# uurl/hivemq-mqtt-tensorflow-kafka-realtime-iot-machine-learning-training-inference

Hardware: AMD Instinct MI355X
Metric: sensor-rows/sec (autoencoder train) + p50 per-event inference µs at 1/2/4/8 MI355X (higher is better)
Workload: dtype bf16

## Files before the change

### hivemq-mqtt-tensorflow-kafka-realtime-iot-machine-learning-training-inference_amd/csrc/include/sml_common.h

```cpp
#pragma once
#include <hip/hip_runtime.h>
#include <stdint.h>

#if defined(SML_KERNEL_CHECKS) && SML_KERNEL_CHECKS
#define SML_DCHECK(cond)                                                           \
  do {                                                                             \
    if (!(cond)) {                                                                 \
      printf("SML_DCHECK failed: %s (%s:%d)\n", #cond, __FILE__, __LINE__);        \
      __builtin_trap();                                                            \
    }                                                                              \
  } while (0)
#else
#define SML_DCHECK(cond) ((void)0)
#endif

namespace sml {

typedef short bf16x4 __attribute__((ext_vector_type(4)));
typedef float f32x4 __attribute__((ext_vector_type(4)));
typedef __bf16 bf16x2_t __attribute__((ext_vector_type(2)));
typedef float f32x2_t __attribute__((ext_vector_type(2)));

enum Act : int { ACT_LINEAR = 0, ACT_RELU = 1, ACT_TANH = 2, ACT_SIGMOID = 3 };

// ... 72 lines not shown
    case ACT_TANH: return 1.0f - h * h;
    case ACT_SIGMOID: return h * (1.0f - h);
    default: return 1.0f;
  }
}

__device__ __forceinline__ bf16x4 identity_b(int c, int g) {
  bf16x4 r;
#pragma unroll
  for (int j = 0; j < 4; ++j) r[j] = (4 * g + j == c) ? (short)0x3F80 : (short)0;
  return r;
}

__device__ __forceinline__ f32x4 transpose_tile(bf16x4 t, bf16x4 ident) {
  f32x4 z = {0.f, 0.f, 0.f, 0.f};
  return mfma16(t, ident, z);
}

__device__ __forceinline__ float xor16(float v, int lane) {
  const unsigned u = __float_as_uint(v);
  const auto r = __builtin_amdgcn_permlane16_swap(u, u, false, false);
  return __uint_as_float(((lane >> 4) & 1) ? r[0] : r[1]);
}
__device__ __forceinline__ float xor32(float v, int lane) {
  const unsigned u = __float_as_uint(v);
  const auto r = __builtin_amdgcn_permlane32_swap(u, u, false, false);
  return __uint_as_float(lane >= 32 ? r[0] : r[1]);
}
__device__ __forceinline__ int xor16i(int v, int lane) { return __float_as_int(xor16(__int_as_float(v), lane)); }
__device__ __forceinline__ int xor32i(int v, int lane) { return __float_as_int(xor32(__int_as_float(v), lane)); }

typedef __attribute__((address_space(3))) bf16x4 lds_bf16x4;

__device__ __forceinline__ int tr_wr_off(int c, int g) { return c * 32 + 8 * (g ^ ((c >> 2) & 3)); }
__device__ __forceinline__ int tr_rd_off(int c, int g) { return (4 * g + (c >> 2)) * 32 + 8 * ((c & 3) ^ g); }
__device__ __forceinline__ bf16x4 lds_transpose(bf16x4 v, char* wave_scratch, int c, int g) {
  lds_bf16x4* wr = (lds_bf16x4*)(wave_scratch + tr_wr_off(c, g));
  *wr = v;
  lds_bf16x4* rd = (lds_bf16x4*)(wave_scratch + tr_rd_off(c, g));
  return __builtin_amdgcn_ds_read_tr16_b64_v4i16(rd);
}

__device__ __forceinline__ float wave_sum(float v) {
#pragma unroll
  for (int o = 32; o > 0; o >>= 1) v += __shfl_xor(v, o, 64);
  return v;
}

}
```

### hivemq-mqtt-tensorflow-kafka-realtime-iot-machine-learning-training-inference_amd/csrc/kernels/ae_fused.hip

```cpp
#include <cstdlib>

#include "sml_common.h"
#include "sml_adam.h"

using namespace sml;

namespace {

constexpr int WAVES = 4;
constexpr int OFF1 = 0, OFF2 = 512, OFF3 = 768, OFF4 = 1024;
constexpr int NPARAM = 1536;
constexpr int NSLOT = 1540;
constexpr int SLAB_BYTES = WAVES * NSLOT * 4;

struct AEArgs {
  const float* x;
  int64_t n;
  int64_t ld;
  const float* scale;
  const float* shift;
  const float* params;
  float* partials;
  int64_t* iter;
  const int64_t* cursor;
// ... 765 lines not shown
  if (s < OFF3) {
    const int in = (s - OFF2) >> 4, out = (s - OFF2) & 15;
    if (out < 7) s2 = s + 8;
    else s1 = -1;
    return;
  }
  const bool l3 = s < OFF4;
  const int base = l3 ? OFF3 : OFF4, w = l3 ? 16 : 32;
  const int in = (s - base) / w, out = (s - base) % w;
  const int pin = in < 7 ? in : (in == 15 ? 7 : -1);
  if (pin < 0 || (l3 && out >= 7)) {
    s1 = -1;
    return;
  }
  if (!l3 && out >= 16) {
    if (out >= 18) {
      s1 = -1;
      return;
    }
    s1 = base + pin * w + 16 + 4 * (out - 16);
    s2 = base + (pin + 8) * w + 16 + 8 + 4 * (out - 16);
    return;
  }
  s1 = base + pin * w + out;
  s2 = base + (pin + 8) * w + out + (l3 ? 8 : 0);
}

__device__ __forceinline__ void tr_write(bf16x4 v, char* slot, int c, int g) {
  *(lds_bf16x4*)(slot + tr_wr_off(c, g)) = v;
}
__device__ __forceinline__ bf16x4 tr_read(char* slot, int c, int g) {
  return __builtin_amdgcn_ds_read_tr16_b64_v4i16((lds_bf16x4*)(slot + tr_rd_off(c, g)));
}

template <int PACK, int DC, bool TP, int TS = 10, int NP = 1, int XP = 0, bool RX = false, bool CM = false,
          bool WA = false, bool RC = true>
__device__ __forceinline__ void train_pair_packed(const AEArgs& a, const FragsP& F, char* scr, int c, int g,
                                                  const f32x4 (&xf)[NP][2][2], const float (&xup)[NP],
                                                  const int (&ix)[NP][2], f32x4 acc1[2], f32x4& acc2, f32x4& acc3,
                                                  f32x4 acc4[2], f32x4& acc2b, f32x4& acc4b, float& sq, float& ab,
                                                  float& corr, float& rows, lds_cc* const* xrow = nullptr,
                                                  lds_cc* const* xupa = nullptr) {
  static_assert(PACK == PACK_REF && DC == 18, "reference model, D = 18 (outputs 16, 17 packed as UP)");
  static_assert(NP == 1 || NP == 2, "one or two pairs per iteration");
  const f32x4 zero4 = {0.f, 0.f, 0.f, 0.f};
  const bf16x4 zb = {0, 0, 0, 0};
  const bool pad_lane = (g == 3);
  const bool lo = c < 8;
  auto stand_in = [](int p, int u) { return TP && p == NP - 1 && u == 1; };
  constexpr bool EW = XP == 1 || XP >= 3, MA = XP >= 1, TRM = XP == 2;
  constexpr bool EB = XP == 4;
  bf16x4 ident;
#pragma unroll
  for (int j = 0; j < 4; ++j) ident[j] = bfbits(4 * g + j == c ? 1.0f : 0.0f);
  auto mfma_tr = [&](bf16x4 v) -> bf16x4 { return pack4(mfma16(v, ident, zero4)); };

  bf16x4 xb0[NP][2], h1b[NP][2], xub[NP];
  f32x4 h1[NP][2], y[NP][2], z1[NP][2], l1s[NP][2];
#pragma unroll
  for (int p = 0; p < NP; ++p) {
#pragma unroll
    for (int u = 0; u < 2; ++u) xb0[p][u] = pack4(xf[p][u][0]);
    xub[p] = pack4(f32x4{xup[p], g == 0 ? 1.0f : 0.0f, 0.f, 0.f});
    if constexpr (EW) {
      tr_write(xb0[p][0], scr + (p * TS + 0) * 512, c, g);
      tr_write(xb0[p][1], scr + (p * TS + 1) * 512, c, g);
      tr_write(xub[p], scr + (p * TS + 2) * 512, c, g);
    }
  }
#pragma unroll
  for (int p = 0; p < NP; ++p) {
    if constexpr (MA) {
      typedef unsigned u32x2 __attribute__((ext_vector_type(2)));
      const unsigned xw = __builtin_bit_cast(u32x2, xub[p])[0];
      const unsigned bias_w = __float_as_uint(g == 0 ? 1.0f : 0.0f);
      const bf16x4 xu0 = __builtin_bit_cast(bf16x4, u32x2{g < 2 ? xw : 0u, 0u});
      const bf16x4 xu1 = __builtin_bit_cast(bf16x4, u32x2{g >= 2 ? xw : bias_w, 0u});
      z1[p][0] = mfma32a(F.w1s, xb0[p][0], xu0, zero4);
      z1[p][1] = mfma32a(F.w1s, xb0[p][1], xu1, zero4);
    } else {
      z1[p][0] = mfma32a(F.w1a[0], xb0[p][0], xub[p], zero4);
      z1[p][1] = mfma32a(F.w1a[1], xub[p], xb0[p][1], zero4);
    }
  }
#pragma unroll
  for (int p = 0; p < NP; ++p)
#pragma unroll
    for (int u = 0; u < 2; ++u) {
#pragma unroll
      for (int i = 0; i < 4; ++i) h1[p][u][i] = tanh_exp2(z1[p][u][i]);
      h1b[p][u] = pack4(h1[p][u]);
      if constexpr (EW) tr_write(h1b[p][u], scr + (p * TS + 3 + u) * 512, c, g);
    }
  auto l1_sign = [&] {
#pragma unroll
    for (int p = 0; p < NP; ++p)
#pragma unroll
      for (int u = 0; u < 2; ++u)
#pragma unroll
        for (int i = 0; i < 4; ++i) l1s[p][u][i] = stand_in(p, u) ? 0.f : __builtin_amdgcn_fmed3f(h1[p][u][i], -a.l1, a.l1);
  };
  if constexpr (!MA) l1_sign();
  f32x4 z2[NP], h2[NP], h3[NP], z3[NP];
  bf16x4 h2b[NP], h3b[NP];
#pragma unroll
  for (int p = 0; p < NP; ++p) z2[p] = mfma32a(F.w2a, h1b[p][0], h1b[p][1], zero4);
#pragma unroll
  for (int p = 0; p < NP; ++p) {
#pragma unroll
    for (int i = 0; i < 4; ++i) h2[p][i] = relu_fast(z2[p][i]);
    h2b[p] = pack4(h2[p]);
    if constexpr (EW) tr_write(h2b[p], scr + (p * TS + 5) * 512, c, g);
  }
#pragma unroll
  for (int p = 0; p < NP; ++p) z3[p] = mfma16(F.w3t, h2b[p], zero4);
#pragma unroll
  for (int p = 0; p < NP; ++p) {
#pragma unroll
    for (int i = 0; i < 4; ++i) h3[p][i] = tanh_exp2(z3[p][i]);
    h3b[p] = pack4(h3[p]);
    if constexpr (EW) tr_write(h3b[p], scr + (p * TS + 6) * 512, c, g);
  }
  f32x4 dz4[NP][2], z4[NP][2], z4u[NP];
  float dz4up[NP], yup[NP];
  f32x4 xl[NP][2];
  float xul[NP];
#pragma unroll
  for (int p = 0; p < NP; ++p) {
    if constexpr (RX) {
      typedef __attribute__((address_space(3))) const float lds_f;
      constexpr int DR = CM ? 14 : 18, SLOTB = 64 * DR + 16;
#pragma unroll
      for (int u = 0; u < 2; ++u) xl[p][u] = ring_row4(xrow[p] + u * SLOTB);
      xul[p] = *(lds_f*)xupa[p];
    } else {
#pragma unroll
      for (int u = 0; u < 2; ++u) xl[p][u] = xf[p][u][0];
      xul[p] = xup[p];
    }
  }
  const float cm_m[3] = {g < 2 ? 0.f : 1.f, g == 1 ? 0.f : 1.f, g == 0 ? 0.f : 1.f};
#pragma unroll
  for (int p = 0; p < NP; ++p) {
#pragma unroll
    for (int u = 0; u < 2; ++u) z4[p][u] = mfma16(F.w4t[u], h3b[p], zero4);
    z4u[p] = mfma16(F.w4u, h3b[p], zero4);
  }
#pragma unroll
  for (int p = 0; p < NP; ++p) {
#pragma unroll
    for (int u = 0; u < 2; ++u)
#pragma unroll
      for (int i = 0; i < 4; ++i) {
        y[p][u][i] = relu_fast(z4[p][u][i]);
        float e = (CM && i < 3) ? fmaf(-xl[p][u][i], cm_m[i], y[p][u][i]) : y[p][u][i] - xl[p][u][i];
        if (stand_in(p, u)) e = 0.f;
        sq = fmaf(e, e, sq);
        dz4[p][u][i] = y[p][u][i] > 0.f ? e : 0.f;
      }
    yup[p] = relu_fast(z4u[p][0]);
    float eup = yup[p] - xul[p];
    if (TP && p == NP - 1) eup = g < 2 ? eup : 0.f;
    sq = fmaf(eup, eup, sq);
    dz4up[p] = yup[p] > 0.f ? eup : 0.f;
  }
  if (WA || a.want_acc) {
#pragma unroll
    for (int p = 0; p < NP; ++p) {
      const int iy = row_argmax_up_pair(y[p][0], y[p][1], yup[p], g);
      const int sel = -(g & 1);
      const int ixs = (ix[p][0] & ~sel) | (ix[p][1] & sel);
      corr += (((TP && p == NP - 1) ? g == 0 : g < 2) && iy == ixs) ? 1.f : 0.f;
    }
  }
  if constexpr (RC) rows += (g == 0) ? (TP ? 2.f * NP - 1.f : 2.f * NP) : 0.f;

  bf16x4 dz4b[NP][2], dz1b[NP][2], dz4bu[NP], dz3b[NP], dz2b[NP];
  f32x4 d3[NP], d2[NP];
#pragma unroll
  for (int p = 0; p < NP; ++p) {
#pragma unroll
    for (int u = 0; u < 2; ++u) dz4b[p][u] = pack4(dz4[p][u]);
    dz4bu[p] = pack4(f32x4{dz4up[p], 0.f, 0.f, 0.f});
    if constexpr (EB) {
      tr_write(dz4b[p][0], scr + (p * TS + 7) * 512, c, g);
      tr_write(dz4b[p][1], scr + (p * TS + 8) * 512, c, g);
      tr_write(dz4bu[p], scr + (p * TS + 9) * 512, c, g);
    }
  }
#pragma unroll
  for (int p = 0; p < NP; ++p) {
    d3[p] = mfma32a(F.w4ba, dz4b[p][0], dz4b[p][1], zero4);
    d3[p] = mfma32a(F.w4bua, dz4bu[p], zb, d3[p]);
  }
#pragma unroll
  for (int p = 0; p < NP; ++p) {
    f32x4 dz3;
#pragma unroll
    for (int i = 0; i < 4; ++i) dz3[i] = d3[p][i] * fmaf(-h3[p][i], h3[p][i], 1.0f);
    dz3b[p] = pack4(dz3);
    if constexpr (EB) tr_write(dz3b[p], scr + (p * TS + 10) * 512, c, g);
  }
#pragma unroll
  for (int p = 0; p < NP; ++p) d2[p] = mfma16(F.w3b, dz3b[p], zero4);
#pragma unroll
  for (int p = 0; p < NP; ++p) {
    f32x4 dz2;
#pragma unroll
    for (int i = 0; i < 4; ++i) dz2[i] = h2[p][i] > 0.f ? d2[p][i] : 0.f;
    dz2b[p] = pack4(dz2);
    if constexpr (EB) tr_write(dz2b[p], scr + (p * TS + 11) * 512, c, g);
  }
  f32x4 d1[NP][2];
  if constexpr (MA) l1_sign();
#pragma unroll
  for (int p = 0; p < NP; ++p)
#pragma unroll
    for (int u = 0; u < 2; ++u) d1[p][u] = mfma16(F.w2b[u], dz2b[p], l1s[p][u]);
#pragma unroll
  for (int p = 0; p < NP; ++p)
#pragma unroll
    for (int u = 0; u < 2; ++u) {
      f32x4 dz1;
#pragma unroll
      for (int i = 0; i < 4; ++i) {
        const float hv = h1[p][u][i];
        if (stand_in(p, u)) {
          dz1[i] = 0.f;
          continue;
        }
        ab += (i == 3 && pad_lane) ? 0.f : fabsf(hv);
        dz1[i] = d1[p][u][i] * fmaf(-hv, hv, 1.0f);
      }
      dz1b[p][u] = pack4(dz1);
    }

  static_assert(TS >= 1 && TS <= 12 && (!EW || TS == (EB ? 12 : 10)), "transpose slots");
  (void)mfma_tr;
#pragma unroll
  for (int p = 0; p < NP; ++p) {
    char* sp = scr + p * TS * 512;
    bf16x4 xr0[2], dz1r[2], h1r[2], dz4r[2], xur, dz4ru, dz2r, h2r, dz3r, h3r;
    if constexpr (EB) {
      h3r = tr_read(sp + 6 * 512, c, g);
      dz4r[0] = tr_read(sp + 7 * 512, c, g);
      dz4r[1] = tr_read(sp + 8 * 512, c, g);
      dz4ru = tr_read(sp + 9 * 512, c, g);
      h2r = tr_read(sp + 5 * 512, c, g);
      dz3r = tr_read(sp + 10 * 512, c, g);
      h1r[0] = tr_read(sp + 3 * 512, c, g);
      h1r[1] = tr_read(sp + 4 * 512, c, g);
      dz2r = tr_read(sp + 11 * 512, c, g);
      xr0[0] = tr_read(sp + 0 * 512, c, g);
      xr0[1] = tr_read(sp + 1 * 512, c, g);
      xur = tr_read(sp + 2 * 512, c, g);
      dz1r[0] = mfma_tr(dz1b[p][0]);
      dz1r[1] = mfma_tr(dz1b[p][1]);
    } else if constexpr (TRM) {
      xr0[0] = mfma_tr(xb0[p][0]);
      xr0[1] = mfma_tr(xb0[p][1]);
      xur = mfma_tr(xub[p]);
      h1r[0] = mfma_tr(h1b[p][0]);
      h1r[1] = mfma_tr(h1b[p][1]);
      h2r = mfma_tr(h2b[p]);
      h3r = mfma_tr(h3b[p]);
      dz4r[0] = mfma_tr(dz4b[p][0]);
      dz4r[1] = mfma_tr(dz4b[p][1]);
      dz4ru = mfma_tr(dz4bu[p]);
      dz3r = mfma_tr(dz3b[p]);
      dz2r = mfma_tr(dz2b[p]);
      dz1r[0] = mfma_tr(dz1b[p][0]);
      dz1r[1] = mfma_tr(dz1b[p][1]);
    } else if constexpr (EW) {
      xr0[0] = tr_read(sp + 0 * 512, c, g);
      xr0[1] = tr_read(sp + 1 * 512, c, g);
      xur = tr_read(sp + 2 * 512, c, g);
// ... 4 lines not shown
      if constexpr (XP == 3) {
        dz4r[0] = mfma_tr(dz4b[p][0]);
        dz4r[1] = mfma_tr(dz4b[p][1]);
        dz4ru = mfma_tr(dz4bu[p]);
        dz3r = mfma_tr(dz3b[p]);
        dz2r = mfma_tr(dz2b[p]);
        dz1r[0] = mfma_tr(dz1b[p][0]);
        dz1r[1] = mfma_tr(dz1b[p][1]);
      } else {
        dz4r[0] = lds_transpose(dz4b[p][0], sp + 7 * 512, c, g);
        dz4r[1] = lds_transpose(dz4b[p][1], sp + 8 * 512, c, g);
        dz4ru = lds_transpose(dz4bu[p], sp + 9 * 512, c, g);
        dz3r = lds_transpose(dz3b[p], sp + 7 * 512, c, g);
        dz2r = lds_transpose(dz2b[p], sp + 8 * 512, c, g);
        dz1r[0] = lds_transpose(dz1b[p][0], sp + 9 * 512, c, g);
        dz1r[1] = lds_transpose(dz1b[p][1], sp + 7 * 512, c, g);
      }
    } else {
      xur = lds_transpose(xub[p], sp + (1 % TS) * 512, c, g);
#pragma unroll
      for (int u = 0; u < 2; ++u) {
        xr0[u] = lds_transpose(xb0[p][u], sp + (0 % TS) * 512, c, g);
        dz1r[u] = lds_transpose(dz1b[p][u], sp + (2 % TS) * 512, c, g);
        h1r[u] = lds_transpose(h1b[p][u], sp + (3 % TS) * 512, c, g);
        dz4r[u] = lds_transpose(dz4b[p][u], sp + (8 % TS) * 512, c, g);
      }
      dz4ru = lds_transpose(dz4bu[p], sp + (9 % TS) * 512, c, g);
      dz2r = lds_transpose(dz2b[p], sp + (4 % TS) * 512, c, g);
      h2r = lds_transpose(h2b[p], sp + (5 % TS) * 512, c, g);
      dz3r = lds_transpose(dz3b[p], sp + (6 % TS) * 512, c, g);
      h3r = lds_transpose(h3b[p], sp + (7 % TS) * 512, c, g);
    }
    acc1[0] = mfma32(xr0[0], xr0[1], dz1r[0], dz1r[1], acc1[0]);
    acc1[1] = mfma32(lo ? xur : zb, (!lo || c == 1) ? xur : zb, dz1r[0], dz1r[1], acc1[1]);
    if constexpr (MA) {
      acc2 = mfma32(h1r[0], h1r[1], lo ? dz2r : zb, lo ? zb : dz2r, acc2);
      acc3 = mfma16(h2r, dz3r, acc3);
      acc4[0] = mfma32(lo ? h3r : zb, lo ? zb : h3r, dz4r[0], dz4r[1], acc4[0]);
    } else {
      acc2 = mfma16(h1r[0], dz2r, acc2);
      acc2b = mfma16(h1r[1], dz2r, acc2b);
      acc3 = mfma16(h2r, dz3r, acc3);
      acc4[0] = mfma16(h3r, dz4r[0], acc4[0]);
      acc4b = mfma16(h3r, dz4r[1], acc4b);
    }
    acc4[1] = mfma16(h3r, dz4ru, acc4[1]);
  }
}

template <int OCC, int ILP = 1>
constexpr int ring_bytes() { return ILP == 3 ? (OCC >= 4 ? 4672 : 7008) : OCC >= 4 ? 3968 : (ILP >= 2 ? 7008 : 6144); }
template <int OCC, int ILP, int PF, int CM = 0>
constexpr int ring_bytes_pf() { return ILP == 3 ? PF * (CM ? 912 : 1168) : ring_bytes<OCC, ILP>(); }

template <int PF, int OCC, int ILP, int TS, int NPW = 1, int CM = 0>
struct AELds {
  static constexpr int SCR = (ILP == 3 ? NPW * TS : 10) * 512;
  static constexpr int NORM_OFF = ILP == 3 ? WAVES * SCR : SLAB_BYTES;
  static constexpr int RING_OFF = NORM_OFF + NORM_BYTES;
  static constexpr int RING = ring_bytes_pf<OCC, ILP, PF, CM>();
  static constexpr int END = RING_OFF + (PF > 0 ? WAVES * RING : 0);
  static constexpr int BYTES = END > SLAB_BYTES ? END : SLAB_BYTES;
};

template <int PACK, bool VEC, int PF, int OCC, int DC = 0, int XM = 0, int ILP = 1, int TS = 10, int NPW = 1,
          int XP = 0, int CM = 0>
__global__ __launch_bounds__(WAVES * 64, OCC) void ae_train_kernel(AEArgs a) {
  constexpr bool FAST = zero_preserving<PACK>();
  constexpr bool CMP = CM != 0;
  static_assert(!CMP || (ILP == 3 && XM == 1 && DC == 18), "compact ring: packed pairs, tile-packed ring, D = 18");
  constexpr int DR = CMP ? 14 : DC;
  using L = AELds<PF, OCC, ILP, (XP == 2 ? 0 : TS), NPW, CM>;
  static_assert(NPW == 1 || ILP == 3, "several pairs per iteration: packed pairs only");
  constexpr int RING = L::RING;
  static_assert(WAVES * (ILP == 3 && NPW == 1 ? TS : 10) * 512 <= SLAB_BYTES,
                "transpose scratch must fit in the slab buffer");
  static_assert(ILP == 3 || TS == 10, "shared transpose slots: packed pairs only");
  static_assert(PF == 0 || CMP || PF * 64 * 17 <= RING, "ring slots must fit the smallest ring tile");
  constexpr bool XA = XM != 0;
  static_assert(XM != 1 || (DC > 0 && PF > 0 && PF * (64 * DR + 16) <= RING), "XA: compile-time D, ring slots + argmax");
  __shared__ __attribute__((aligned(16))) float smem[L::BYTES / 4];
  const int lane = threadIdx.x & 63;
  const int wid = threadIdx.x >> 6;
  const int c = lane & 15, g = lane >> 4;
  char* scr = reinterpret_cast<char*>(smem) + wid * L::SCR;
  const char* norm = reinterpret_cast<const char*>(smem) + L::NORM_OFF;
  if (a.cursor) {
    a.x += a.cursor[0] * a.ld;
    if (XM == 1) a.xpack += (a.cursor[0] >> 4) * (int64_t)(64 * (CMP ? DR : a.D) + 16);
  }

  if (a.iter && blockIdx.x == 0 && threadIdx.x == 0) a.iter[0] += 1;
  if (threadIdx.x < 64) {
    const int f = threadIdx.x & 31;
    smem[L::NORM_OFF / 4 + threadIdx.x] = threadIdx.x < 32 ? norm_scale(a, f) : norm_shift(a, f);
  }

  Frags F;
  FragsP FP;
  if constexpr (ILP == 3)
    load_frags_packed<CMP>(a, c, g, FP);
  else
    load_frags<FAST, FAST && prescaled_tanh<PACK>(), FAST && inject_bias_slots<PACK>()>(a, c, g, F, true);
  const float pad1 = (g == 3) ? 1.0f : 0.0f;
  __syncthreads();

  f32x4 acc1[2], acc2, acc3, acc4[2], acc2b, acc4b;
  const f32x4 zero4 = {0.f, 0.f, 0.f, 0.f};
  acc1[0] = acc1[1] = acc2 = acc3 = acc4[0] = acc4[1] = acc2b = acc4b = zero4;
  float sq = 0.f, ab = 0.f, corr = 0.f, rows = 0.f;

  const int64_t nfull = a.n >> 4;
  const int64_t stride = (int64_t)gridDim.x * WAVES;
  const int64_t first = (int64_t)blockIdx.x * WAVES + wid;
  if constexpr (PF > 0) {
    const int slotb = 64 * (DR > 0 ? DR : a.D) + (XM == 1 ? 16 : 0);
    constexpr int NV = 2;
    const int nl2 = (slotb - 1024) >> 4;
    const int uwid = __builtin_amdgcn_readfirstlane(wid);
    const int ring_off = L::RING_OFF + uwid * RING;
    const unsigned ring_lds =
        (unsigned)(uintptr_t)((__attribute__((address_space(3))) char*)smem) + ring_off;
    const char* ring = reinterpret_cast<const char*>(smem) + ring_off;
    const int64_t ufirst = (int64_t)blockIdx.x * WAVES + uwid;
    const unsigned voff = lane * 16;
    __builtin_amdgcn_s_waitcnt(0x0F70);
    if (nfull > 0) {
      auto issue = [&](int64_t tt, int slot) {
        tt = tt < nfull ? tt : nfull - 1;
        const char* src = XM == 1 ? reinterpret_cast<const char*>(a.xpack) + tt * slotb
                                  : reinterpret_cast<const char*>(a.x + tt * 16 * a.ld);
        const unsigned dst = ring_lds + slot * slotb;
        glds16(src, voff, dst);
        if (lane < nl2) glds16(src + 1024, voff, dst + 1024);
      };
      constexpr int CH = XM == 3 ? 8 : 1;
      auto next_tile = [&](int64_t t) -> int64_t {
// ... 57 lines not shown
            ring_tile(2 * slot, xf[0], ix[0]);
            ring_tile(2 * slot + 1, xf[1], ix[1]);
            xup = ring_up(2 * slot);
            if constexpr (XM == 0) {
              typedef __attribute__((address_space(3))) const f32x4 lds_f4;
              typedef __attribute__((address_space(3))) const float lds_f;
              const f32x4 nsc = *(lds_f4*)(norm + 16 * g), nsh = *(lds_f4*)(norm + 128 + 16 * g);
              const int fu = 4 * (16 + (g & 1));
              const float usc = *(lds_f*)(norm + fu), ush = *(lds_f*)(norm + 128 + fu);
#pragma unroll
              for (int u = 0; u < 2; ++u)
#pragma unroll
                for (int j = 0; j < 4; ++j) xf[u][0][j] = fmaf(xf[u][0][j], nsc[j], nsh[j]);
              xup = fmaf(xup, usc, ush);
              ix[0] = ix[1] = a.want_acc ? row_argmax_up_pair_signed(xf[0][0], xf[1][0], xup, g) : -1;
            }
          };
          (void)load_pair;
          if constexpr (NPW == 1 && XM == 1 && PS == 2) {
            const unsigned np32 = (unsigned)npairs, st32 = (unsigned)stride, uf32 = (unsigned)ufirst;
            const unsigned ntrip = __builtin_amdgcn_readfirstlane(uf32 < np32 ? (np32 - 1u - uf32) / st32 + 1u : 0u);
            unsigned pq = uf32;
            auto issue_next = [&](int ps) {
              issue_pair_at(pq < np32 ? pq : np32 - 1u, ps);
              pq += st32;
            };
#pragma unroll
            for (int k = 0; k < PS - 1; ++k) issue_next(k);
            lds_cc* rowb = (lds_cc*)(ring + row_off);
            lds_cc* upb = (lds_cc*)(ring + up_off);
            lds_cc* axb = (lds_cc*)(ring + (slotb - 16) + c);
            asm volatile("" : "+v"(rowb), "+v"(upb));
            asm volatile("" : "+v"(axb));
            auto trip = [&](auto slot) {
              constexpr int rs = decltype(slot)::value, ws = (rs + PS - 1) % PS;
              issue_next(ws);
              asm volatile("s_waitcnt vmcnt(%0)" ::"n"(NVP * (PS - 1)) : "memory");
              typedef __attribute__((address_space(3))) const unsigned char lds_u8;
              typedef __attribute__((address_space(3))) const float lds_f;
              f32x4 xf[1][2][2];
              float xup[1];
              int ix[1][2];
              lds_cc* const xr[1] = {rowb + 2 * rs * slotb};
              lds_cc* const xu[1] = {upb + 2 * rs * slotb};
#pragma unroll
              for (int u = 0; u < 2; ++u) {
                xf[0][u][0] = ring_row4(xr[0] + u * slotb);
                xf[0][u][1] = f32x4{0.f, 0.f, 0.f, 0.f};
                ix[0][u] = (int)*(lds_u8*)(axb + (2 * rs + u) * slotb);
              }
              xup[0] = *(lds_f*)xu[0];
              constexpr bool RX = OCC >= 4;
              train_pair_packed<PACK, DC, false, TS, 1, XP, RX, CMP, true, false>(
                  a, FP, scr, c, g, xf, xup, ix, acc1, acc2, acc3, acc4, acc2b, acc4b, sq, ab, corr, rows, xr, xu);
            };
            for (unsigned k = ntrip; k > 0; k -= PS) {
              trip(RingSlot<0>{});
              if (k == 1) break;
              trip(RingSlot<1>{});
            }
            rows += (g == 0) ? 2.f * (float)ntrip : 0.f;
            asm volatile("s_waitcnt vmcnt(0)" ::: "memory");
          } else {
          int64_t pp = ufirst;
#pragma unroll
          for (int k = 0; k < PS - NPW; ++k) {
            issue_pair(pp, k);
            pp += stride;
          }
          int rs = 0, ws = PS - NPW;
          int64_t pi = ufirst;
          for (; pi + (NPW - 1) * stride < npairs; pi += NPW * stride) {
#pragma unroll
            for (int k = 0; k < NPW; ++k) {
              issue_pair(pp, ws);
              pp += stride;
              ws = ws + 1 == PS ? 0 : ws + 1;
            }
            asm volatile("s_waitcnt vmcnt(%0)" ::"n"(NVP * (PS - NPW)) : "memory");
            f32x4 xf[NPW][2][2];
            float xup[NPW];
            int ix[NPW][2];
            lds_cc* xr[NPW];
            lds_cc* xu[NPW];
#pragma unroll
            for (int k = 0; k < NPW; ++k) {
              load_pair(rs, xf[k], xup[k], ix[k]);
// ... 90 lines not shown
      asm volatile("s_waitcnt vmcnt(0)" ::: "memory");
      }
    }
  } else {
    f32x4 xnext[2];
    if (first < nfull) fetch_x<VEC>(a, first * 16 + c, g, xnext);
    for (int64_t t = first; t < nfull; t += stride) {
      f32x4 xf[2], sc[2], sh[2];
      norm_lds(norm, g, sc, sh);
#pragma unroll
      for (int s = 0; s < 2; ++s)
#pragma unroll
        for (int j = 0; j < 4; ++j) xf[s][j] = fmaf(xnext[s][j], sc[s][j], sh[s][j]);
      if (t + stride < nfull) fetch_x<VEC>(a, (t + stride) * 16 + c, g, xnext);
      train_tile<PACK, FAST, false>(a, F, scr, c, g, lane, true, xf, pad1, acc1, acc2, acc3, acc4, sq, ab, corr,
                                    rows);
    }
  }
  if (ILP != 3 && (a.n & 15) && first == nfull % stride) {
    const int64_t r = nfull * 16 + c;
    const bool valid = r < a.n;
    f32x4 xf[2], sc[2], sh[2];
    fetch_x<VEC>(a, r, g, xf);
    norm_lds(norm, g, sc, sh);
#pragma unroll
    for (int s = 0; s < 2; ++s)
#pragma unroll
      for (int j = 0; j < 4; ++j) xf[s][j] = valid ? fmaf(xf[s][j], sc[s][j], sh[s][j]) : 0.f;
    train_tile<PACK, FAST, true>(a, F, scr, c, g, lane, valid, xf, pad1, acc1, acc2, acc3, acc4, sq, ab, corr, rows);
  }

  __syncthreads();
  float* my = smem + wid * NSLOT;
  if constexpr (ILP == 3) {
    if constexpr (XP == 0) {
      acc2 = c < 8 ? acc2 : acc2b;
      acc4[0] = g < 2 ? acc4[0] : acc4b;
    }
  }
#pragma unroll
  for (int i = 0; i < 4; ++i) {
    const int m = 4 * g + i;
    my[OFF1 + m * 16 + c] = acc1[0][i];
    my[OFF1 + (16 + m) * 16 + c] = acc1[1][i];
    my[OFF2 + m * 16 + c] = acc2[i];
    my[OFF3 + m * 16 + c] = acc3[i];
    my[OFF4 + m * 32 + c] = acc4[0][i] * (2.0f / (float)a.D);
    my[OFF4 + m * 32 + 16 + c] = acc4[1][i] * (2.0f / (float)a.D);
  }
  sq = wave_sum(sq);
  ab = wave_sum(ab);
  corr = wave_sum(corr);
  rows = wave_sum(rows);
  if (lane == 0) {
    my[NPARAM + 0] = sq;
    my[NPARAM + 1] = ab;
    my[NPARAM + 2] = corr;
    my[NPARAM + 3] = rows;
  }
  __syncthreads();
  float* out = a.partials + (int64_t)blockIdx.x * NSLOT;
  for (int s = threadIdx.x; s < NSLOT; s += WAVES * 64) {
    if constexpr (ILP == 3) {
      int s1, s2;
      packed_fold_src<CMP>(s, s1, s2);
      float v = 0.f;
#pragma unroll
      for (int w = 0; w < WAVES; ++w) {
        if (s1 >= 0) v += smem[w * NSLOT + s1];
        if (s2 >= 0) v += smem[w * NSLOT + s2];
      }
      out[s] = v;
    } else {
      float v = smem[s];
#pragma unroll
      for (int w = 1; w < WAVES; ++w) v += smem[w * NSLOT + s];
      out[s] = v;
    }
  }
}

// ... 275 lines not shown
    const float t = (float)iter[0];
    lr_t = sml::adam_lr_t(hp.lr, hp.beta1, hp.beta2, t);
  }
#pragma unroll
  for (int e = 0; e < 4; ++e)
    adam_one(tot[e], quad * 4 + e, nparam, grad_out, params, m, v, lr_t, hp, gscale, metrics_acc, flags);
}
}

namespace sml {

static bool ring_pf_enabled() {
  static const bool on = [] {
    const char* e = getenv("SML_AE_RING");
    return !(e && e[0] == '0');
  }();
  return on;
}

static int train_ilp() {
  const char* e = getenv("SML_AE_ILP");
  return (e && (e[0] == '1' || e[0] == '2')) ? e[0] - '0' : 3;
}
static bool direct_pairs() {
  const char* e = getenv("SML_AE_DIRECT_PAIRS");
  return !(e && e[0] == '0');
}
static int pair_occ() {
  const char* e = getenv("SML_AE_PAIR_OCC");
  return (e && (e[0] == '2' || e[0] == '3' || e[0] == '4')) ? e[0] - '0' : 4;
}
static int pair_xp() {
  const char* e = getenv("SML_AE_PAIR_XP");
  return (e && e[0] >= '0' && e[0] <= '4') ? e[0] - '0' : 4;
}
static int train_occupancy() {
  const char* e = getenv("SML_AE_OCC");
  return (e && e[0] == '3') ? 3 : 4;
}
int ae_train_blocks_per_cu() { return 8; }
static int device_cus() {
  static const int cus = [] {
    int dev = 0, n = 0;
    if (hipGetDevice(&dev) != hipSuccess || hipDeviceGetAttribute(&n, hipDeviceAttributeMultiprocessorCount, dev) !=
                                                 hipSuccess || n <= 0)
      return 256;
    return n;
  }();
  return cus;
}

int ae_nslot() { return NSLOT; }
int ae_nparam() { return NPARAM; }
int ae_waves_per_block() { return WAVES; }

struct LastVariant {
  const void* fn = nullptr;
  int xp = -1, ts = -1;
};
static thread_local LastVariant last_variant;
void ae_train_last_variant(int out[3]) {
  out[0] = last_variant.xp;
  out[1] = last_variant.ts;
  out[2] = -1;
  hipFuncAttributes attr{};
  if (last_variant.fn && hipFuncGetAttributes(&attr, last_variant.fn) == hipSuccess) out[2] = (int)attr.sharedSizeBytes;
}
// ... 44 lines not shown
  auto launch_noted = [&](void (*kern)(AEArgs), int xp_, int ts_) {
    last_variant = LastVariant{reinterpret_cast<const void*>(kern), xp_, ts_};
    hipLaunchKernelGGL(kern, gd, bd, 0, stream, a);
  };
  if (pack == PACK_REF) {
    const bool xa_ok = xpack != nullptr && want_acc && (n & 15) == 0 &&
                       ((reinterpret_cast<uintptr_t>(xpack) & 15) == 0);
    static const int probe = [] {
      const char* e = std::getenv("SML_AE_XPROBE");
      return e ? std::atoi(e) : 0;
    }();
    if ((n >> 5) >= (int64_t(1) << 30)) return hipErrorInvalidValue;
    const bool pairs_ok = ((n >> 4) & 1) == 0 && train_ilp() == 3 && dims[1] <= 15 && dims[2] <= 7 && dims[3] <= 7;
    const bool full = xpack_live == 0 || (D <= 31 && xpack_live == (1u << D) - 1u);
    const bool cm = !full && D == 18 && xpack_live == kLiveCardata;
    if (xpack != nullptr && !full && !cm) return hipErrorInvalidValue;
    const bool xpack_used = xa_ok && ring_ok && D == 18 && (cm ? pairs_ok : (train_ilp() == 2 || pairs_ok || occ == 4));
    if (xpack != nullptr && !xpack_used && (probe < 2 || cm)) return hipErrorInvalidValue;
    if (ring_ok && occ == 4 && D == 18 && want_acc && probe == 2)
      hipLaunchKernelGGL((ae_train_kernel<PACK_REF, true, 3, 4, 18, 2>), gd, bd, 0, stream, a);
    else if (ring_ok && occ == 4 && D == 18 && want_acc && probe == 3)
      hipLaunchKernelGGL((ae_train_kernel<PACK_REF, true, 3, 4, 18, 3>), gd, bd, 0, stream, a);
    else if (ring_ok && D == 18 && xa_ok && train_ilp() == 2) {
      pair_grid();
      hipLaunchKernelGGL((ae_train_kernel<PACK_REF, true, 6, 3, 18, 1, 2>), gd, bd, 0, stream, a);
    } else if (ring_ok && D == 18 && xa_ok && ((n >> 4) & 1) == 0 && train_ilp() == 3 && dims[1] <= 15 &&
               dims[2] <= 7 && dims[3] <= 7) {
      const int po = pair_occ();
      pair_grid(po);
      const int xp = pair_xp();
      if (cm) {
        if (po == 2)
          hipLaunchKernelGGL((ae_train_kernel<PACK_REF, true, 8, 2, 18, 1, 3, 10, 2, 0, 1>), gd, bd, 0, stream, a);
        else if (po == 4 && xp == 4)
          launch_noted(ae_train_kernel<PACK_REF, true, 4, 4, 18, 1, 3, 12, 1, 4, 1>, 4, 12);
        else if (po == 4 && xp >= 2)
          launch_noted(ae_train_kernel<PACK_REF, true, 4, 4, 18, 1, 3, 10, 1, 3, 1>, 3, 10);
        else if (xp >= 3)
          hipLaunchKernelGGL((ae_train_kernel<PACK_REF, true, 6, 3, 18, 1, 3, 10, 1, 3, 1>), gd, bd, 0, stream, a);
        else if (po == 4)
          hipLaunchKernelGGL((ae_train_kernel<PACK_REF, true, 4, 4, 18, 1, 3, 10, 1, 1, 1>), gd, bd, 0, stream, a);
        else if (xp == 1)
          hipLaunchKernelGGL((ae_train_kernel<PACK_REF, true, 6, 3, 18, 1, 3, 10, 1, 1, 1>), gd, bd, 0, stream, a);
        else if (xp == 2)
          hipLaunchKernelGGL((ae_train_kernel<PACK_REF, true, 6, 3, 18, 1, 3, 10, 1, 2, 1>), gd, bd, 0, stream, a);
        else
          hipLaunchKernelGGL((ae_train_kernel<PACK_REF, true, 6, 3, 18, 1, 3, 10, 1, 0, 1>), gd, bd, 0, stream, a);
      } else if (po == 2)
        hipLaunchKernelGGL((ae_train_kernel<PACK_REF, true, 8, 2, 18, 1, 3, 10, 2>), gd, bd, 0, stream, a);
      else if (po == 4 && xp >= 2)
        hipLaunchKernelGGL((ae_train_kernel<PACK_REF, true, 4, 4, 18, 1, 3, 10, 1, 3>), gd, bd, 0, stream, a);
      else if (xp >= 3)
        hipLaunchKernelGGL((ae_train_kernel<PACK_REF, true, 6, 3, 18, 1, 3, 10, 1, 3>), gd, bd, 0, stream, a);
      else if (po == 4)
        hipLaunchKernelGGL((ae_train_kernel<PACK_REF, true, 4, 4, 18, 1, 3, 10, 1, 1>), gd, bd, 0, stream, a);
      else if (xp == 1)
        hipLaunchKernelGGL((ae_train_kernel<PACK_REF, true, 6, 3, 18, 1, 3, 10, 1, 1>), gd, bd, 0, stream, a);
      else if (xp == 2)
        hipLaunchKernelGGL((ae_train_kernel<PACK_REF, true, 6, 3, 18, 1, 3, 10, 1, 2>), gd, bd, 0, stream, a);
      else
        hipLaunchKernelGGL((ae_train_kernel<PACK_REF, true, 6, 3, 18, 1, 3>), gd, bd, 0, stream, a);
    }
    else if (ring_ok && occ == 4 && D == 18 && xa_ok)
      hipLaunchKernelGGL((ae_train_kernel<PACK_REF, true, 3, 4, 18, 1>), gd, bd, 0, stream, a);
    else if (ring_ok && D == 18 && xpack == nullptr && (n & 31) == 0 && train_ilp() == 3 && direct_pairs() &&
             dims[1] <= 15 && dims[2] <= 7 && dims[3] <= 7) {
// ... 81 lines not shown
```

Measured before the change: 56.30 billion.

## Use masked transpose reads from a shared zero/identity cell to drop lane selects

Adds an XP=5 training variant where the weight-gradient MFMAs take their operands from per-lane precomputed LDS read addresses. For half the lanes these point at a shared cell that holds zeros and a unit value, so each transpose read returns the already-masked operand. This replaces the per-lane select-with-zero logic around the transposed xu, dz2 and h3 tiles. It rearranges scratch slot assignments, adds a small mask-cell region to LDS initialised once per block, and makes this variant the default. The cost is extra LDS reads and footprint plus more address registers per lane.

```diff
diff --git a/hivemq-mqtt-tensorflow-kafka-realtime-iot-machine-learning-training-inference_amd/csrc/include/sml_common.h b/hivemq-mqtt-tensorflow-kafka-realtime-iot-machine-learning-training-inference_amd/csrc/include/sml_common.h
--- a/hivemq-mqtt-tensorflow-kafka-realtime-iot-machine-learning-training-inference_amd/csrc/include/sml_common.h
+++ b/hivemq-mqtt-tensorflow-kafka-realtime-iot-machine-learning-training-inference_amd/csrc/include/sml_common.h
@@ -128,8 +128,14 @@
 
 typedef __attribute__((address_space(3))) bf16x4 lds_bf16x4;
 
-__device__ __forceinline__ int tr_wr_off(int c, int g) { return c * 32 + 8 * (g ^ ((c >> 2) & 3)); }
-__device__ __forceinline__ int tr_rd_off(int c, int g) { return (4 * g + (c >> 2)) * 32 + 8 * ((c & 3) ^ g); }
+__host__ __device__ __forceinline__ int tr_wr_off(int c, int g) { return c * 32 + 8 * (g ^ ((c >> 2) & 3)); }
+__host__ __device__ __forceinline__ int tr_rd_off(int c, int g) { return (4 * g + (c >> 2)) * 32 + 8 * ((c & 3) ^ g); }
+__host__ __device__ __forceinline__ int tr_rd_off_half(int c, int g, int half, int cells) {
+  const int p = c & 3;
+  return (p >> 1) == half ? tr_rd_off(c, g) : cells + 8 * p;
+}
+constexpr int TR_MASK_CELL_BYTES = 2 * 512 + 32;
+__host__ __device__ __forceinline__ unsigned tr_mask_cell_word(int i) { return i == 0 ? 0x3F800000u : 0u; }
 __device__ __forceinline__ bf16x4 lds_transpose(bf16x4 v, char* wave_scratch, int c, int g) {
   lds_bf16x4* wr = (lds_bf16x4*)(wave_scratch + tr_wr_off(c, g));
   *wr = v;
diff --git a/hivemq-mqtt-tensorflow-kafka-realtime-iot-machine-learning-training-inference_amd/csrc/kernels/ae_fused.hip b/hivemq-mqtt-tensorflow-kafka-realtime-iot-machine-learning-training-inference_amd/csrc/kernels/ae_fused.hip
--- a/hivemq-mqtt-tensorflow-kafka-realtime-iot-machine-learning-training-inference_amd/csrc/kernels/ae_fused.hip
+++ b/hivemq-mqtt-tensorflow-kafka-realtime-iot-machine-learning-training-inference_amd/csrc/kernels/ae_fused.hip
@@ -821,6 +821,10 @@
 __device__ __forceinline__ bf16x4 tr_read(char* slot, int c, int g) {
   return __builtin_amdgcn_ds_read_tr16_b64_v4i16((lds_bf16x4*)(slot + tr_rd_off(c, g)));
 }
+__device__ __forceinline__ bf16x4 tr_read_at(lds_cc* lane_addr) {
+  return __builtin_amdgcn_ds_read_tr16_b64_v4i16((lds_bf16x4*)lane_addr);
+}
+constexpr int MASK_SLOT0 = 9, MASK_CELL_BYTES = TR_MASK_CELL_BYTES;
 
 template <int PACK, int DC, bool TP, int TS = 10, int NP = 1, int XP = 0, bool RX = false, bool CM = false,
           bool WA = false, bool RC = true>
@@ -829,16 +833,23 @@
                                                   const int (&ix)[NP][2], f32x4 acc1[2], f32x4& acc2, f32x4& acc3,
                                                   f32x4 acc4[2], f32x4& acc2b, f32x4& acc4b, float& sq, float& ab,
                                                   float& corr, float& rows, lds_cc* const* xrow = nullptr,
-                                                  lds_cc* const* xupa = nullptr) {
+                                                  lds_cc* const* xupa = nullptr, lds_cc* rd_lo = nullptr,
+                                                  lds_cc* rd_hi = nullptr) {
   static_assert(PACK == PACK_REF && DC == 18, "reference model, D = 18 (outputs 16, 17 packed as UP)");
   static_assert(NP == 1 || NP == 2, "one or two pairs per iteration");
   const f32x4 zero4 = {0.f, 0.f, 0.f, 0.f};
   const bf16x4 zb = {0, 0, 0, 0};
   const bool pad_lane = (g == 3);
   const bool lo = c < 8;
+  const float pad_m = pad_lane ? 0.f : 1.f;
   auto stand_in = [](int p, int u) { return TP && p == NP - 1 && u == 1; };
   constexpr bool EW = XP == 1 || XP >= 3, MA = XP >= 1, TRM = XP == 2;
-  constexpr bool EB = XP == 4;
+  constexpr bool EB = XP >= 4;
+  constexpr bool MR = XP == 5;
+  constexpr int S_XU = MR ? 9 : 2, S_H1 = MR ? 2 : 3, S_H2 = MR ? 4 : 5, S_H3 = MR ? 10 : 6, S_DZ4 = MR ? 5 : 7,
+                S_DZ4U = MR ? 7 : 9, S_DZ3 = MR ? 8 : 10, S_DZ2 = 11;
+  static_assert(!MR || (NP == 1 && S_XU == MASK_SLOT0 && S_H3 == MASK_SLOT0 + 1 && S_DZ2 == MASK_SLOT0 + 2),
+                "masked reads: one pair per wave, the masked slots where the kernel put their cells");
   bf16x4 ident;
 #pragma unroll
   for (int j = 0; j < 4; ++j) ident[j] = bfbits(4 * g + j == c ? 1.0f : 0.0f);
@@ -854,7 +865,7 @@
     if constexpr (EW) {
       tr_write(xb0[p][0], scr + (p * TS + 0) * 512, c, g);
       tr_write(xb0[p][1], scr + (p * TS + 1) * 512, c, g);
-      tr_write(xub[p], scr + (p * TS + 2) * 512, c, g);
+      tr_write(xub[p], scr + (p * TS + S_XU) * 512, c, g);
     }
   }
 #pragma unroll
@@ -879,7 +890,7 @@
 #pragma unroll
       for (int i = 0; i < 4; ++i) h1[p][u][i] = tanh_exp2(z1[p][u][i]);
       h1b[p][u] = pack4(h1[p][u]);
-      if constexpr (EW) tr_write(h1b[p][u], scr + (p * TS + 3 + u) * 512, c, g);
+      if constexpr (EW) tr_write(h1b[p][u], scr + (p * TS + S_H1 + u) * 512, c, g);
     }
   auto l1_sign = [&] {
 #pragma unroll
@@ -899,7 +910,7 @@
 #pragma unroll
     for (int i = 0; i < 4; ++i) h2[p][i] = relu_fast(z2[p][i]);
     h2b[p] = pack4(h2[p]);
-    if constexpr (EW) tr_write(h2b[p], scr + (p * TS + 5) * 512, c, g);
+    if constexpr (EW) tr_write(h2b[p], scr + (p * TS + S_H2) * 512, c, g);
   }
 #pragma unroll
   for (int p = 0; p < NP; ++p) z3[p] = mfma16(F.w3t, h2b[p], zero4);
@@ -908,7 +919,7 @@
 #pragma unroll
     for (int i = 0; i < 4; ++i) h3[p][i] = tanh_exp2(z3[p][i]);
     h3b[p] = pack4(h3[p]);
-    if constexpr (EW) tr_write(h3b[p], scr + (p * TS + 6) * 512, c, g);
+    if constexpr (EW) tr_write(h3b[p], scr + (p * TS + S_H3) * 512, c, g);
   }
   f32x4 dz4[NP][2], z4[NP][2], z4u[NP];
   float dz4up[NP], yup[NP];
@@ -972,9 +983,9 @@
     for (int u = 0; u < 2; ++u) dz4b[p][u] = pack4(dz4[p][u]);
     dz4bu[p] = pack4(f32x4{dz4up[p], 0.f, 0.f, 0.f});
     if constexpr (EB) {
-      tr_write(dz4b[p][0], scr + (p * TS + 7) * 512, c, g);
-      tr_write(dz4b[p][1], scr + (p * TS + 8) * 512, c, g);
-      tr_write(dz4bu[p], scr + (p * TS + 9) * 512, c, g);
+      tr_write(dz4b[p][0], scr + (p * TS + S_DZ4) * 512, c, g);
+      tr_write(dz4b[p][1], scr + (p * TS + S_DZ4 + 1) * 512, c, g);
+      tr_write(dz4bu[p], scr + (p * TS + S_DZ4U) * 512, c, g);
     }
   }
 #pragma unroll
@@ -988,7 +999,7 @@
 #pragma unroll
     for (int i = 0; i < 4; ++i) dz3[i] = d3[p][i] * fmaf(-h3[p][i], h3[p][i], 1.0f);
     dz3b[p] = pack4(dz3);
-    if constexpr (EB) tr_write(dz3b[p], scr + (p * TS + 10) * 512, c, g);
+    if constexpr (EB) tr_write(dz3b[p], scr + (p * TS + S_DZ3) * 512, c, g);
   }
 #pragma unroll
   for (int p = 0; p < NP; ++p) d2[p] = mfma16(F.w3b, dz3b[p], zero4);
@@ -998,7 +1009,7 @@
 #pragma unroll
     for (int i = 0; i < 4; ++i) dz2[i] = h2[p][i] > 0.f ? d2[p][i] : 0.f;
     dz2b[p] = pack4(dz2);
-    if constexpr (EB) tr_write(dz2b[p], scr + (p * TS + 11) * 512, c, g);
+    if constexpr (EB) tr_write(dz2b[p], scr + (p * TS + S_DZ2) * 512, c, g);
   }
   f32x4 d1[NP][2];
   if constexpr (MA) l1_sign();
@@ -1018,7 +1029,10 @@
           dz1[i] = 0.f;
           continue;
         }
-        ab += (i == 3 && pad_lane) ? 0.f : fabsf(hv);
+        if (MR && i == 3)
+          ab = fmaf(fabsf(hv), pad_m, ab);
+        else
+          ab += (i == 3 && pad_lane) ? 0.f : fabsf(hv);
         dz1[i] = d1[p][u][i] * fmaf(-hv, hv, 1.0f);
       }
       dz1b[p][u] = pack4(dz1);
@@ -1030,7 +1044,27 @@
   for (int p = 0; p < NP; ++p) {
     char* sp = scr + p * TS * 512;
     bf16x4 xr0[2], dz1r[2], h1r[2], dz4r[2], xur, dz4ru, dz2r, h2r, dz3r, h3r;
-    if constexpr (EB) {
+    bf16x4 xur_m[2], dz2r_m[2], h3r_m[2];
+    if constexpr (MR) {
+      h3r = tr_read(sp + S_H3 * 512, c, g);
+      h3r_m[0] = tr_read_at(rd_lo + S_H3 * 512);
+      h3r_m[1] = tr_read_at(rd_hi + S_H3 * 512);
+      dz4r[0] = tr_read(sp + S_DZ4 * 512, c, g);
+      dz4r[1] = tr_read(sp + (S_DZ4 + 1) * 512, c, g);
+      dz4ru = tr_read(sp + S_DZ4U * 512, c, g);
+      h2r = tr_read(sp + S_H2 * 512, c, g);
+      dz3r = tr_read(sp + S_DZ3 * 512, c, g);
+      h1r[0] = tr_read(sp + S_H1 * 512, c, g);
+      h1r[1] = tr_read(sp + (S_H1 + 1) * 512, c, g);
+      dz2r_m[0] = tr_read_at(rd_lo + S_DZ2 * 512);
+      dz2r_m[1] = tr_read_at(rd_hi + S_DZ2 * 512);
+      xr0[0] = tr_read(sp + 0 * 512, c, g);
+      xr0[1] = tr_read(sp + 1 * 512, c, g);
+      xur_m[0] = tr_read_at(rd_lo + S_XU * 512);
+      xur_m[1] = tr_read_at(rd_hi + S_XU * 512);
+      dz1r[0] = mfma_tr(dz1b[p][0]);
+      dz1r[1] = mfma_tr(dz1b[p][1]);
+    } else if constexpr (EB) {
       h3r = tr_read(sp + 6 * 512, c, g);
       dz4r[0] = tr_read(sp + 7 * 512, c, g);
       dz4r[1] = tr_read(sp + 8 * 512, c, g);
@@ -1101,8 +1135,15 @@
       h3r = lds_transpose(h3b[p], sp + (7 % TS) * 512, c, g);
     }
     acc1[0] = mfma32(xr0[0], xr0[1], dz1r[0], dz1r[1], acc1[0]);
-    acc1[1] = mfma32(lo ? xur : zb, (!lo || c == 1) ? xur : zb, dz1r[0], dz1r[1], acc1[1]);
-    if constexpr (MA) {
+    if constexpr (MR)
+      acc1[1] = mfma32(xur_m[0], xur_m[1], dz1r[0], dz1r[1], acc1[1]);
+    else
+      acc1[1] = mfma32(lo ? xur : zb, (!lo || c == 1) ? xur : zb, dz1r[0], dz1r[1], acc1[1]);
+    if constexpr (MR) {
+      acc2 = mfma32(h1r[0], h1r[1], dz2r_m[0], dz2r_m[1], acc2);
+      acc3 = mfma16(h2r, dz3r, acc3);
+      acc4[0] = mfma32(h3r_m[0], h3r_m[1], dz4r[0], dz4r[1], acc4[0]);
+    } else if constexpr (MA) {
       acc2 = mfma32(h1r[0], h1r[1], lo ? dz2r : zb, lo ? zb : dz2r, acc2);
       acc3 = mfma16(h2r, dz3r, acc3);
       acc4[0] = mfma32(lo ? h3r : zb, lo ? zb : h3r, dz4r[0], dz4r[1], acc4[0]);
@@ -1122,13 +1163,14 @@
 template <int OCC, int ILP, int PF, int CM = 0>
 constexpr int ring_bytes_pf() { return ILP == 3 ? PF * (CM ? 912 : 1168) : ring_bytes<OCC, ILP>(); }
 
-template <int PF, int OCC, int ILP, int TS, int NPW = 1, int CM = 0>
+template <int PF, int OCC, int ILP, int TS, int NPW = 1, int CM = 0, int MC = 0>
 struct AELds {
   static constexpr int SCR = (ILP == 3 ? NPW * TS : 10) * 512;
   static constexpr int NORM_OFF = ILP == 3 ? WAVES * SCR : SLAB_BYTES;
   static constexpr int RING_OFF = NORM_OFF + NORM_BYTES;
   static constexpr int RING = ring_bytes_pf<OCC, ILP, PF, CM>();
-  static constexpr int END = RING_OFF + (PF > 0 ? WAVES * RING : 0);
+  static constexpr int CELLS_OFF = RING_OFF + (PF > 0 ? WAVES * RING : 0);
+  static constexpr int END = CELLS_OFF + MC;
   static constexpr int BYTES = END > SLAB_BYTES ? END : SLAB_BYTES;
 };
 
@@ -1139,7 +1181,10 @@
   constexpr bool CMP = CM != 0;
   static_assert(!CMP || (ILP == 3 && XM == 1 && DC == 18), "compact ring: packed pairs, tile-packed ring, D = 18");
   constexpr int DR = CMP ? 14 : DC;
-  using L = AELds<PF, OCC, ILP, (XP == 2 ? 0 : TS), NPW, CM>;
+  constexpr bool MR = XP == 5;
+  static_assert(!MR || (ILP == 3 && XM == 1 && NPW == 1 && PF == 4 && TS == 12), "XP 5: the unrolled two-slot pair loop");
+  using L = AELds<PF, OCC, ILP, (XP == 2 ? 0 : TS), NPW, CM, MR ? MASK_CELL_BYTES : 0>;
+  static_assert(L::BYTES <= 40960 || OCC < 4, "four workgroups per CU");
   static_assert(NPW == 1 || ILP == 3, "several pairs per iteration: packed pairs only");
   constexpr int RING = L::RING;
   static_assert(WAVES * (ILP == 3 && NPW == 1 ? TS : 10) * 512 <= SLAB_BYTES,
@@ -1172,6 +1217,10 @@
   else
     load_frags<FAST, FAST && prescaled_tanh<PACK>(), FAST && inject_bias_slots<PACK>()>(a, c, g, F, true);
   const float pad1 = (g == 3) ? 1.0f : 0.0f;
+  if constexpr (MR) {
+    for (int i = threadIdx.x; i < MASK_CELL_BYTES / 4; i += WAVES * 64)
+      smem[L::CELLS_OFF / 4 + i] = __uint_as_float(tr_mask_cell_word(i));
+  }
   __syncthreads();
 
   f32x4 acc1[2], acc2, acc3, acc4[2], acc2b, acc4b;
@@ -1295,6 +1344,14 @@
             lds_cc* axb = (lds_cc*)(ring + (slotb - 16) + c);
             asm volatile("" : "+v"(rowb), "+v"(upb));
             asm volatile("" : "+v"(axb));
+            lds_cc* rd_lo = nullptr;
+            lds_cc* rd_hi = nullptr;
+            if constexpr (MR) {
+              const int cells = L::CELLS_OFF - MASK_SLOT0 * 512 - wid * L::SCR;
+              rd_lo = (lds_cc*)scr + tr_rd_off_half(c, g, 0, cells);
+              rd_hi = (lds_cc*)scr + tr_rd_off_half(c, g, 1, cells);
+              asm volatile("" : "+v"(rd_lo), "+v"(rd_hi));
+            }
             auto trip = [&](auto slot) {
               constexpr int rs = decltype(slot)::value, ws = (rs + PS - 1) % PS;
               issue_next(ws);
@@ -1315,7 +1372,8 @@
               xup[0] = *(lds_f*)xu[0];
               constexpr bool RX = OCC >= 4;
               train_pair_packed<PACK, DC, false, TS, 1, XP, RX, CMP, true, false>(
-                  a, FP, scr, c, g, xf, xup, ix, acc1, acc2, acc3, acc4, acc2b, acc4b, sq, ab, corr, rows, xr, xu);
+                  a, FP, scr, c, g, xf, xup, ix, acc1, acc2, acc3, acc4, acc2b, acc4b, sq, ab, corr, rows, xr, xu, rd_lo,
+                  rd_hi);
             };
             for (unsigned k = ntrip; k > 0; k -= PS) {
               trip(RingSlot<0>{});
@@ -1472,21 +1530,28 @@
 
   __syncthreads();
   float* my = smem + wid * NSLOT;
+  int ce = c, ge = g;
+  if constexpr (MR) {
+    int le = threadIdx.x & 63;
+    asm volatile("" : "+v"(le));
+    ce = le & 15;
+    ge = le >> 4;
+  }
   if constexpr (ILP == 3) {
     if constexpr (XP == 0) {
-      acc2 = c < 8 ? acc2 : acc2b;
-      acc4[0] = g < 2 ? acc4[0] : acc4b;
+      acc2 = ce < 8 ? acc2 : acc2b;
+      acc4[0] = ge < 2 ? acc4[0] : acc4b;
     }
   }
 #pragma unroll
   for (int i = 0; i < 4; ++i) {
-    const int m = 4 * g + i;
-    my[OFF1 + m * 16 + c] = acc1[0][i];
-    my[OFF1 + (16 + m) * 16 + c] = acc1[1][i];
-    my[OFF2 + m * 16 + c] = acc2[i];
-    my[OFF3 + m * 16 + c] = acc3[i];
-    my[OFF4 + m * 32 + c] = acc4[0][i] * (2.0f / (float)a.D);
-    my[OFF4 + m * 32 + 16 + c] = acc4[1][i] * (2.0f / (float)a.D);
+    const int m = 4 * ge + i;
+    my[OFF1 + m * 16 + ce] = acc1[0][i];
+    my[OFF1 + (16 + m) * 16 + ce] = acc1[1][i];
+    my[OFF2 + m * 16 + ce] = acc2[i];
+    my[OFF3 + m * 16 + ce] = acc3[i];
+    my[OFF4 + m * 32 + ce] = acc4[0][i] * (2.0f / (float)a.D);
+    my[OFF4 + m * 32 + 16 + ce] = acc4[1][i] * (2.0f / (float)a.D);
   }
   sq = wave_sum(sq);
   ab = wave_sum(ab);
@@ -1828,7 +1893,7 @@
 }
 static int pair_xp() {
   const char* e = getenv("SML_AE_PAIR_XP");
-  return (e && e[0] >= '0' && e[0] <= '4') ? e[0] - '0' : 4;
+  return (e && e[0] >= '0' && e[0] <= '5') ? e[0] - '0' : 5;
 }
 static int train_occupancy() {
   const char* e = getenv("SML_AE_OCC");
@@ -1939,6 +2004,8 @@
       if (cm) {
         if (po == 2)
           hipLaunchKernelGGL((ae_train_kernel<PACK_REF, true, 8, 2, 18, 1, 3, 10, 2, 0, 1>), gd, bd, 0, stream, a);
+        else if (po == 4 && xp == 5)
+          launch_noted(ae_train_kernel<PACK_REF, true, 4, 4, 18, 1, 3, 12, 1, 5, 1>, 5, 12);
         else if (po == 4 && xp == 4)
           launch_noted(ae_train_kernel<PACK_REF, true, 4, 4, 18, 1, 3, 12, 1, 4, 1>, 4, 12);
         else if (po == 4 && xp >= 2)
```

Result: faster. 57.00 billion, median of 6 (+1.2%).
